# thangvubk/SoftGroup

Hardware: AMD Instinct MI355X
Metric: scans/sec ScanNet-v2-like inference (softgroup_scannet.yaml, full forward_test) (higher is better)
Workload: dtype f32

## Files before the change

### softgroup_amd/csrc/bfs.hip

```cpp
#include <stdlib.h>

#include <atomic>
#include <map>
#include <mutex>
#include <utility>

#include "common.h"
#include "scan.h"

namespace sg {

constexpr int kCap = SG_BALLQUERY_MAX_NEIGHBORS;
constexpr int kEmitThreads = 512;
constexpr int kEmitWaves = kEmitThreads / 64;

#define SG_LD(p) __hip_atomic_load((p), __ATOMIC_RELAXED, __HIP_MEMORY_SCOPE_AGENT)
#define SG_ST(p, v) __hip_atomic_store((p), (v), __ATOMIC_RELAXED, __HIP_MEMORY_SCOPE_AGENT)

struct BfsWs {
  int32_t *parent, *lab, *size, *cid, *coff, *owner, *seeds, *ebase, *wcnt, *asym_nodes;
  int4 *label;
  int2 *erec;
  int32_t *counters;
  void *scan_ws;
  size_t scan_bytes;
  int32_t *big_stage[2];
  unsigned long long *big_rec[2];
};

constexpr int kBigFastWgs = 16;
constexpr int kBigSlice = 8192;
constexpr int kBigClusterMin = 16384;
inline bool big_fast_on() {
  const char *e = getenv("SG_BFS_BIG_FAST");
  return !(e && atoi(e) == 0);
}
inline int thin_levels_on() {
  const char *e = getenv("SG_BFS_THIN");
  return e ? atoi(e) : 0;
}
inline bool big_local_on() {
  const char *e = getenv("SG_BFS_BIG_LOCAL");
  return !(e && atoi(e) == 0);
}
inline size_t big_stage_entries(int n) {
  return n > kBigClusterMin && big_fast_on() ? static_cast<size_t>(n) + static_cast<size_t>(kBigFastWgs) * kBigSlice : 0;
}

static bool bfs_carve(void *ws, size_t ws_bytes, int n, int64_t n_edges, BfsWs *w) {
  Workspace a(ws, ws_bytes);
  const size_t nn = static_cast<size_t>(n > 0 ? n : 1);
  w->parent = a.take<int32_t>(nn);
  w->lab = a.take<int32_t>(nn);
  w->label = a.take<int4>(nn);
  w->size = a.take<int32_t>(nn);
  w->cid = a.take<int32_t>(nn);
  w->coff = a.take<int32_t>(nn);
  w->owner = a.take<int32_t>(nn);
  w->seeds = a.take<int32_t>(nn);
  w->ebase = a.take<int32_t>(nn);
  w->wcnt = a.take<int32_t>(nn);
  w->asym_nodes = a.take<int32_t>(nn);
  w->counters = a.take<int32_t>(64);
  w->scan_bytes = scan_workspace_bytes(n);
  w->scan_ws = a.take<char>(w->scan_bytes);
  w->erec = a.take<int2>(static_cast<size_t>(n_edges > 0 ? n_edges : 1));
  bool ok = w->scan_ws != nullptr && w->erec != nullptr;
  const size_t be = big_stage_entries(n);
  for (int i = 0; i < 2; ++i) {
    w->big_stage[i] = be ? a.take<int32_t>(be) : nullptr;
    w->big_rec[i] = be ? a.take<unsigned long long>(be) : nullptr;
    ok = ok && (be == 0 || (w->big_stage[i] != nullptr && w->big_rec[i] != nullptr));
// ... 4 lines not shown
__device__ __forceinline__ int uf_find(int32_t *parent, int x) {
  int cur = SG_LD(&parent[x]);
  if (cur != x) {
    int prev = x, next;
    while (cur > (next = SG_LD(&parent[cur]))) {
      SG_ST(&parent[prev], next);
      prev = cur;
      cur = next;
    }
  }
  return cur;
}

__device__ __forceinline__ void uf_union(int32_t *parent, int a, int b) {
  while (a != b) {
    if (a < b) { const int t = a; a = b; b = t; }
    const int old = atomicCAS(&parent[a], a, b);
    if (old == a) return;
    a = uf_find(parent, old);
    b = uf_find(parent, b);
  }
}

__device__ __forceinline__ bool list_has_sorted(const int32_t *__restrict__ lst, int len, int key) {
  int lo = 0, hi = len;
  while (lo < hi) {
    const int mid = (lo + hi) >> 1;
    const int v = lst[mid];
    if (v < key) lo = mid + 1; else hi = mid;
  }
  return lo < len && lst[lo] == key;
}

__global__ void __launch_bounds__(256) bfs_init_kernel(int n, int32_t *parent, int32_t *size,
                                                      int32_t *owner) {
  const int i = blockIdx.x * 256 + threadIdx.x;
  if (i < n) {
    parent[i] = i;
    size[i] = 0;
    owner[i] = 0x7fffffff;
  }
}

constexpr int kSample = 2;
template <int SAMPLE, int G>
__global__ void __launch_bounds__(256) bfs_union_kernel(const int32_t *__restrict__ idx,
                                                       const int32_t *__restrict__ start_len, int n,
                                                       int lists_sorted, int radius_lists,
                                                       int32_t *parent, int32_t *asym_nodes,
                                                       int32_t *counters) {
  constexpr int kNodes = 64 / G;
  const int wave = threadIdx.x >> 6, lane = group_lane<G>(), sub = (threadIdx.x & 63) / G;
  for (int u0 = (blockIdx.x * 4 + wave) * kNodes; u0 < n; u0 += gridDim.x * 4 * kNodes) {
    const int u = u0 + sub;
    const bool live = G == 64 || u < n;
    const int st = live ? start_len[2 * u] : 0, ln_all = live ? start_len[2 * u + 1] : 0;
    const int ln = SAMPLE ? min(ln_all, kSample) : ln_all;
    const bool u_capped = ln_all >= kCap;
    bool any_asym = false;
    const int ru = SAMPLE || !live ? -1 : SG_LD(&parent[u]);
    for (int p0 = 0; p0 < ln; p0 += G) {
      const int p = p0 + lane;
      const int v = p < ln ? idx[st + p] : u;
      bool sym = true;
      if (v != u) {
        const int vst = start_len[2 * v], vln = start_len[2 * v + 1];
        if (!radius_lists || u_capped || vln >= kCap) {
          if (lists_sorted) {
            sym = list_has_sorted(idx + vst, vln, u);
          } else {
            sym = false;
            for (int j = 0; j < vln; ++j)
              if (idx[vst + j] == u) { sym = true; break; }
          }
        }
        if (sym) {
          if (v < u && (SAMPLE || SG_LD(&parent[v]) != ru)) uf_union(parent, uf_find(parent, u), uf_find(parent, v));
        }
      }
      any_asym |= !sym;
    }
    if (!SAMPLE && group_any<G>(any_asym)) {
      if (lane == 0) asym_nodes[atomicAdd(&counters[0], 1)] = u;
    }
  }
}

__global__ void __launch_bounds__(256) bfs_hook_min_kernel(const int32_t *__restrict__ idx,
                                                          const int32_t *__restrict__ start_len, int n,
                                                          int lists_sorted, int radius_lists, int32_t *parent) {
  const int u = blockIdx.x * 256 + threadIdx.x;
  if (u >= n) return;
  const int st = start_len[2 * u], ln = start_len[2 * u + 1];
  if (ln == 0 || !lists_sorted) return;
  const int v = idx[st];
  if (v >= u) return;
  if (!radius_lists || ln >= kCap || start_len[2 * v + 1] >= kCap)
    if (!list_has_sorted(idx + start_len[2 * v], start_len[2 * v + 1], u)) return;
  parent[u] = v;
}
__global__ void __launch_bounds__(256) bfs_compress_kernel(int n, int32_t *parent) {
  const int i = blockIdx.x * 256 + threadIdx.x;
  if (i < n) SG_ST(&parent[i], uf_find(parent, i));
}

__global__ void __launch_bounds__(256) bfs_flatten_kernel(int n, int32_t *parent, int32_t *lab) {
  const int i = blockIdx.x * 256 + threadIdx.x;
  if (i >= n) return;
  int r = i;
  while (true) {
    const int p = SG_LD(&parent[r]);
    if (p == r) break;
    r = p;
  }
  lab[i] = r;
}
__global__ void __launch_bounds__(256) bfs_store_root_kernel(int n, const int32_t *__restrict__ lab,
                                                            int32_t *__restrict__ parent) {
  const int i = blockIdx.x * 256 + threadIdx.x;
  if (i < n) parent[i] = lab[i];
}

template <int G>
__global__ void __launch_bounds__(256) bfs_propagate_kernel(const int32_t *__restrict__ idx,
                                                           const int32_t *__restrict__ start_len,
                                                           const int32_t *__restrict__ asym_nodes,
                                                           int n_asym,
                                                           const int32_t *__restrict__ root_of,
                                                           int32_t *lab, int32_t *counters) {
  const int lane = group_lane<G>();
  for (int a = (blockIdx.x * 256 + threadIdx.x) / G; a < n_asym; a += (gridDim.x * 256) / G) {
    const int u = asym_nodes[a];
    const int ru = root_of[u];
    const int st = start_len[2 * u], ln = start_len[2 * u + 1];
    for (int p = lane; p < ln; p += G) {
      const int rv = root_of[idx[st + p]];
      if (rv == ru) continue;
      const int lu = SG_LD(&lab[ru]);
      if (lu < SG_LD(&lab[rv])) {
        if (atomicMin(&lab[rv], lu) > lu) SG_ST(&counters[1], 1);
      }
    }
  }
}

__global__ void __launch_bounds__(256) bfs_label_kernel(int n, const int32_t *__restrict__ root_of,
                                                       const int32_t *__restrict__ lab,
                                                       const int32_t *__restrict__ start_len,
                                                       int4 *__restrict__ node_rec, int32_t *size) {
  const int i = blockIdx.x * 256 + threadIdx.x;
  const bool valid = i < n;
  const int l = valid ? lab[root_of[i]] : -1;
  int rank = 0, peers = 0, my_leader = threadIdx.x & 63;
// ... 67 lines not shown
      erec[rv.z + p] = rt.x == rv.x ? make_int2(min(rt.y, 0xfffe) | (rt.w << 16), rt.z)
                                    : make_int2(0xffff, 0);
    }
  }
}

__device__ __forceinline__ void lds_prefetch_b32(const void *gsrc, unsigned lds_dst) {
  unsigned keep;
  asm volatile("s_mov_b32 %0, m0\n\ts_mov_b32 m0, %2\n\ts_nop 0\n\tglobal_load_lds_dword %1, off\n\t"
               "s_mov_b32 m0, %0"
               : "=&s"(keep) : "v"(gsrc), "s"(lds_dst) : "memory");
}

__device__ __forceinline__ int wg_excl_scan(int v, int *lds, int *total) {
  const int w = threadIdx.x >> 6, l = threadIdx.x & 63;
  const int incl = wave_incl_scan(v);
  if (l == 63) lds[w] = incl;
  __syncthreads();
  int carry = 0, tot = 0;
#pragma unroll
  for (int i = 0; i < kEmitWaves; ++i) {
    const int x = lds[i];
    if (i < w) carry += x;
    tot += x;
  }
  __syncthreads();
  *total = tot;
  return carry + incl - v;
}

constexpr int kOwnCap = 16384;
constexpr int kFrontChunk = 1024;
constexpr int kE2 = 4096;
constexpr int kThinIter = 8;
constexpr int kThinEdges = 64 * kThinIter;
static_assert(kThinEdges <= kFrontChunk, "a thin level's winners must fit the LDS frontier");

__global__ void __launch_bounds__(kEmitThreads) bfs_emit_kernel(
    const int32_t *__restrict__ idx, const int32_t *__restrict__ start_len,
    const int4 *__restrict__ node_rec, const int2 *__restrict__ erec,
    const int32_t *__restrict__ seeds, const int32_t *__restrict__ cluster_offsets, int n_cluster,
    int32_t *owner_g, int32_t *cluster_idxs, int32_t *stats, int skip_above, int only_above,
    const int32_t *gate ,
    int thin_mode ) {
  const bool thin_on = thin_mode != 0, thin_prefetch = thin_mode == 2;
  if (gate != nullptr && SG_LD(gate) == 0) return;
  __shared__ int lds_scan[kEmitWaves];
  __shared__ int own_lds[kOwnCap];
  __shared__ int f_st[2][kFrontChunk], f_ln[2][kFrontChunk];
  __shared__ int f_eb[kFrontChunk], f_wc[kFrontChunk];
  __shared__ unsigned short ebuf[kE2];
  __shared__ int e_st[kE2], e_g[kE2];
  __shared__ unsigned short e_ln[kE2];
  __shared__ int pf_sink[kEmitThreads];
  __shared__ unsigned char thin_map[kThinEdges];
  __shared__ int thin_state[8];
  const int wave = threadIdx.x >> 6, lane = threadIdx.x & 63;
  const unsigned pf_dst = __builtin_amdgcn_readfirstlane(
      static_cast<unsigned>(reinterpret_cast<uintptr_t>(pf_sink + wave * 64)));
  static_assert(sizeof(int2) == 8, "edge records are 8 bytes: 16 per 128-byte line");
  for (int c = blockIdx.x; c < n_cluster; c += gridDim.x) {
    const int seed = seeds[c];
    const int off = cluster_offsets[c];
    const int size = cluster_offsets[c + 1] - off;
    if (size > skip_above || size <= only_above) continue;
    const bool own_in_lds = size <= kOwnCap;
    int32_t *Q = cluster_idxs + 2LL * off;
    if (own_in_lds)
      for (int i = threadIdx.x; i < size; i += kEmitThreads) own_lds[i] = 0x7fffffff;
    __syncthreads();
    if (threadIdx.x == 0) {
      const int4 rec = node_rec[seed];
      SG_ST(&Q[0], c);
      SG_ST(&Q[1], seed);
      if (own_in_lds) own_lds[rec.y] = -1; else SG_ST(&owner_g[seed], -1);
      f_st[0][0] = rec.z;
      f_ln[0][0] = rec.w;
    }
    asm volatile("s_waitcnt vmcnt(0)" ::: "memory");
    __syncthreads();
    auto rec2 = [&](int v) -> int2 { return *reinterpret_cast<const int2 *>(node_rec + v); };
    auto claim = [&](int v, int pos) {
      const int2 ll = rec2(v);
      if (ll.x != seed) return;
      if (own_in_lds) { if (own_lds[ll.y] > pos) atomicMin(&own_lds[ll.y], pos); }
      else if (SG_LD(&owner_g[v]) > pos) atomicMin(&owner_g[v], pos);
    };
    auto owner_of = [&](int v) -> int {
      const int2 ll = rec2(v);
      if (ll.x != seed) return -2;
      return own_in_lds ? own_lds[ll.y] : SG_LD(&owner_g[v]);
    };
    auto mark_done = [&](int v) {
      if (own_in_lds) own_lds[rec2(v).y] = -1; else SG_ST(&owner_g[v], -1);
    };
    int head = 0, tail = 1;
    int n_fast = 0, n_gen = 0, sum_e = 0, max_l = 0;
    int conv_lo = -1;
    auto convert_pending = [&]() {
      if (conv_lo < 0) return;
      for (int o = conv_lo + threadIdx.x; o < tail; o += kEmitThreads)
        SG_ST(&Q[2 * o + 1], idx[SG_LD(&Q[2 * o + 1])]);
      conv_lo = -1;
      asm volatile("s_waitcnt vmcnt(0)" ::: "memory");
      __syncthreads();
    };
    int cur = 0;
    bool in_lds = true;
    bool thin_ok = thin_on;
    while (head < tail) {
      const int L = tail - head;
      if (thin_ok && own_in_lds && in_lds && L <= 64) {
        if (wave == 0) {
          int h = head, t = tail, cu = cur, cl = conv_lo, levels = 0, edges = 0;
          while (true) {
            const int Lw = t - h;
            if (Lw <= 0 || Lw > 64) break;
            const int ln = lane < Lw ? f_ln[cu][lane] : 0;
            const int incl = wave_incl_scan(ln);
            const int E = __builtin_amdgcn_readlane(incl, 63);
            if (E > kThinEdges) break;
            const int eb = incl - ln;
            if (lane < Lw) f_eb[lane] = eb;
            for (int q = 0; q < Lw; ++q) {
              const int ln_q = __builtin_amdgcn_readlane(ln, q), eb_q = __builtin_amdgcn_readlane(eb, q);
              for (int p = lane; p < ln_q; p += 64) thin_map[eb_q + p] = static_cast<unsigned char>(q);
            }
            int2 r[kThinIter];
            int g[kThinIter];
#pragma unroll
            for (int j = 0; j < kThinIter; ++j) {
              const int e = j * 64 + lane;
              g[j] = 0;
              r[j] = make_int2(0xffff, 0);
              if (e < E) {
                const int q = thin_map[e];
                g[j] = f_st[cu][q] + (e - f_eb[q]);
                r[j] = erec[g[j]];
              }
            }
#pragma unroll
            for (int j = 0; j < kThinIter; ++j) {
              const int e = j * 64 + lane;
              const int slot = r[j].x & 0xffff;
              if (e < E && slot != 0xffff) {
                const int cur_owner = own_lds[slot];
                if (cur_owner > e) atomicMin(&own_lds[slot], e);
                if (thin_prefetch && cur_owner >= 0) {
                  const int tl = r[j].x >> 16;
                  const char *first = reinterpret_cast<const char *>(erec + r[j].y);
                  const char *last = reinterpret_cast<const char *>(erec + r[j].y + max(tl, 1) - 1);
                  const uintptr_t l0 = reinterpret_cast<uintptr_t>(first) & ~static_cast<uintptr_t>(127);
                  const int nlines = static_cast<int>(((reinterpret_cast<uintptr_t>(last) & ~static_cast<uintptr_t>(127)) - l0) >> 7) + 1;
                  for (int k = 0; k < 4; ++k)
                    if (k < nlines) lds_prefetch_b32(reinterpret_cast<const void *>(l0 + 128u * k), pf_dst);
                }
              }
            }
            const int nxt = cu ^ 1;
            int t_new = 0;
#pragma unroll
            for (int j = 0; j < kThinIter; ++j) {
              const int e = j * 64 + lane;
              const int slot = r[j].x & 0xffff;
              const bool win = e < E && slot != 0xffff && own_lds[slot] == e;
              const uint64_t bal = __ballot(win);
              if (win) {
                const int oo = t_new + mask_prefix(bal);
                SG_ST(&Q[2 * (t + oo)], c);
                SG_ST(&Q[2 * (t + oo) + 1], g[j]);
                f_st[nxt][oo] = r[j].y;
                f_ln[nxt][oo] = r[j].x >> 16;
                own_lds[slot] = -1;
              }
              t_new += __popcll(bal);
            }
            if (cl < 0 && t_new > 0) cl = t;
            h = t;
            t += t_new;
            cu = nxt;
            ++levels;
            edges += E;
          }
          asm volatile("s_waitcnt vmcnt(0)" ::: "memory");
          if (lane == 0) {
            thin_state[0] = h; thin_state[1] = t; thin_state[2] = cu; thin_state[3] = cl;
            thin_state[4] = levels; thin_state[5] = edges;
          }
        }
        __syncthreads();
        const int levels = thin_state[4];
        head = thin_state[0];
        tail = thin_state[1];
        cur = thin_state[2];
        conv_lo = thin_state[3];
        n_fast += levels;
        sum_e += thin_state[5];
        max_l = max(max_l, L);
        __syncthreads();
        in_lds = true;
        thin_ok = false;
        if (levels > 0) continue;
      }
      thin_ok = thin_on;
      int E = -1;
      if (in_lds && L <= kFrontChunk) {
        int carry = 0;
        for (int b0 = 0; b0 < L; b0 += kEmitThreads) {
          const int q = b0 + threadIdx.x;
          const int ln = q < L ? f_ln[cur][q] : 0;
          int tot;
          const int ex = wg_excl_scan(ln, lds_scan, &tot);
          if (q < L) f_eb[q] = carry + ex;
          carry += tot;
        }
        __syncthreads();
        E = carry;
      }
      if (E >= 0 && E <= kE2) {
        ++n_fast; sum_e += E; max_l = max(max_l, L);
        for (int e = threadIdx.x; e < E; e += kEmitThreads) {
          int lo = 0, hi = L;
          while (hi - lo > 1) {
            const int mid = (lo + hi) >> 1;
            if (f_eb[mid] <= e) lo = mid; else hi = mid;
          }
          const int g = f_st[cur][lo] + (e - f_eb[lo]);
          const int2 r = erec[g];
          const unsigned short slot = static_cast<unsigned short>(r.x & 0xffff);
          ebuf[e] = slot;
          e_g[e] = g;
          e_st[e] = r.y;
          e_ln[e] = static_cast<unsigned short>(r.x >> 16);
          if (slot != 0xffffu) {
            if (own_in_lds) {
              const int cur_owner = own_lds[slot];
              if (cur_owner > e) atomicMin(&own_lds[slot], e);
              if (cur_owner >= 0) {
                const int tl = r.x >> 16;
                const char *first = reinterpret_cast<const char *>(erec + r.y);
                const char *last = reinterpret_cast<const char *>(erec + r.y + max(tl, 1) - 1);
                const uintptr_t l0 = reinterpret_cast<uintptr_t>(first) & ~static_cast<uintptr_t>(127);
                const int nlines = static_cast<int>(((reinterpret_cast<uintptr_t>(last) & ~static_cast<uintptr_t>(127)) - l0) >> 7) + 1;
                for (int j = 0; j < 4; ++j)
                  if (j < nlines) lds_prefetch_b32(reinterpret_cast<const void *>(l0 + 128u * j), pf_dst);
              }
            } else {
              const int v = idx[g];
              if (SG_LD(&owner_g[v]) > e) atomicMin(&owner_g[v], e);
            }
          }
        }
        if (!own_in_lds) asm volatile("s_waitcnt vmcnt(0)" ::: "memory");
        __syncthreads();
        const int nxt = cur ^ 1;
        int t_new = 0;
        for (int b0 = 0; b0 < E; b0 += kEmitThreads) {
          const int e = b0 + threadIdx.x;
          unsigned short slot = 0xffffu;
          bool win = false;
          int v = 0;
          if (e < E) {
            slot = ebuf[e];
            if (slot != 0xffffu) {
              if (own_in_lds) {
                win = own_lds[slot] == e;
              } else {
                v = idx[e_g[e]];
                win = SG_LD(&owner_g[v]) == e;
              }
            }
          }
          int tot;
          const int oo = t_new + wg_excl_scan(win ? 1 : 0, lds_scan, &tot);
          if (win) {
            SG_ST(&Q[2 * (tail + oo)], c);
            SG_ST(&Q[2 * (tail + oo) + 1], e_g[e]);
            if (oo < kFrontChunk) {
              f_st[nxt][oo] = e_st[e];
              f_ln[nxt][oo] = e_ln[e];
            }
            if (own_in_lds) own_lds[slot] = -1; else SG_ST(&owner_g[v], -1);
          }
          t_new += tot;
        }
        if (conv_lo < 0 && t_new > 0) conv_lo = tail;
        if (!own_in_lds) asm volatile("s_waitcnt vmcnt(0)" ::: "memory");
        __syncthreads();
        head = tail;
        tail += t_new;
        cur = nxt;
        in_lds = t_new <= kFrontChunk;
        continue;
      }
      ++n_gen; max_l = max(max_l, L);
      convert_pending();
      auto stage = [&](int ch, int carry_in) -> int {
        const int q0 = ch * kFrontChunk, cnt = min(kFrontChunk, L - q0);
        int carry = carry_in;
        for (int b0 = 0; b0 < cnt; b0 += kEmitThreads) {
          const int q = b0 + threadIdx.x;
          int ln = 0;
          if (q < cnt) {
            const int4 rec = node_rec[SG_LD(&Q[2 * (head + q0 + q) + 1])];
            f_st[0][q] = rec.z;
            ln = rec.w;
            f_ln[0][q] = ln;
          }
          int tot;
          const int ex = wg_excl_scan(ln, lds_scan, &tot);
          if (q < cnt) f_eb[q] = carry + ex;
          carry += tot;
        }
        __syncthreads();
        return carry;
      };
      const int n_chunks = (L + kFrontChunk - 1) / kFrontChunk;
      int carry = 0;
      for (int ch = 0; ch < n_chunks; ++ch) {
        carry = stage(ch, carry);
        const int cnt = min(kFrontChunk, L - ch * kFrontChunk);
        for (int q = wave; q < cnt; q += kEmitWaves) {
          const int st = f_st[0][q], ln = f_ln[0][q], base = f_eb[q];
          for (int p = lane; p < ln; p += 64) claim(idx[st + p], base + p);
        }
        __syncthreads();
      }
      asm volatile("s_waitcnt vmcnt(0)" ::: "memory");
      __syncthreads();
      int appended = 0;
      carry = 0;
      for (int ch = 0; ch < n_chunks; ++ch) {
        carry = stage(ch, carry);
        const int cnt = min(kFrontChunk, L - ch * kFrontChunk);
        for (int q = wave; q < cnt; q += kEmitWaves) {
          const int st = f_st[0][q], ln = f_ln[0][q], base = f_eb[q];
          int wins = 0;
          for (int p0 = 0; p0 < ln; p0 += 64) {
            const int p = p0 + lane;
            wins += __popcll(__ballot(p < ln && owner_of(idx[st + p]) == base + p));
          }
          if (lane == 0) f_wc[q] = wins;
        }
        __syncthreads();
        int chunk_new = 0;
        for (int b0 = 0; b0 < cnt; b0 += kEmitThreads) {
          const int q = b0 + threadIdx.x;
          const int w_ = q < cnt ? f_wc[q] : 0;
          int tot;
          const int ex = wg_excl_scan(w_, lds_scan, &tot);
          if (q < cnt) f_wc[q] = chunk_new + ex;
          chunk_new += tot;
        }
        __syncthreads();
        for (int q = wave; q < cnt; q += kEmitWaves) {
          const int st = f_st[0][q], ln = f_ln[0][q], base = f_eb[q];
          int obase = tail + appended + f_wc[q];
          for (int p0 = 0; p0 < ln; p0 += 64) {
            const int p = p0 + lane;
            int v = 0;
            bool win = false;
            if (p < ln) {
              v = idx[st + p];
              win = owner_of(v) == base + p;
            }
            const uint64_t bal = __ballot(win);
            if (win) {
              const int o = obase + mask_prefix(bal);
              SG_ST(&Q[2 * o], c);
              SG_ST(&Q[2 * o + 1], v);
            }
            obase += __popcll(bal);
          }
        }
        appended += chunk_new;
        __syncthreads();
      }
      asm volatile("s_waitcnt vmcnt(0)" ::: "memory");
      __syncthreads();
      for (int o = tail + threadIdx.x; o < tail + appended; o += kEmitThreads)
        mark_done(SG_LD(&Q[2 * o + 1]));
      const bool keep = own_in_lds && appended <= kFrontChunk;
      if (keep)
        for (int o = threadIdx.x; o < appended; o += kEmitThreads) {
          const int4 rec = node_rec[SG_LD(&Q[2 * (tail + o) + 1])];
          f_st[0][o] = rec.z;
          f_ln[0][o] = rec.w;
        }
      asm volatile("s_waitcnt vmcnt(0)" ::: "memory");
      __syncthreads();
      head = tail;
      tail += appended;
      cur = 0;
      in_lds = keep;
    }
    convert_pending();
    if (stats && threadIdx.x == 0 && c < 256) {
      stats[c * 8 + 0] = size; stats[c * 8 + 1] = n_fast; stats[c * 8 + 2] = n_gen;
      stats[c * 8 + 3] = sum_e; stats[c * 8 + 4] = max_l;
    }
    __syncthreads();
  }
}


constexpr int kBigWgsMax = 256;
constexpr int kBigMin = kOwnCap;
constexpr int kBigNodes = 1024;
constexpr int kBigEdges = 8192;
constexpr int kBigDirectDegree = 32;
static_assert(kBigSlice == kBigEdges && kBigClusterMin == kBigMin && kBfsGiantMin == kBigMin, "staging sizes follow the kernel's constants");
static_assert(kBigNodes <= 65535, "c_j holds node indices of a range as 16-bit");

__device__ __forceinline__ bool big_barrier(int32_t *bar, int &epoch, int32_t *fail, int *lds_flag) {
  asm volatile("s_waitcnt vmcnt(0)" ::: "memory");
  __syncthreads();
  if (threadIdx.x == 0) {
    __hip_atomic_fetch_add(bar, 1, __ATOMIC_RELAXED, __HIP_MEMORY_SCOPE_AGENT);
    const int target = (epoch + 1) * static_cast<int>(gridDim.x);
    unsigned spins = 0;
    int ok = 1;
    while (__hip_atomic_load(bar, __ATOMIC_RELAXED, __HIP_MEMORY_SCOPE_AGENT) < target) {
      __builtin_amdgcn_s_sleep(1);
      if ((++spins & 1023u) == 0u) {
        if (spins > (1u << 24) || __hip_atomic_load(fail, __ATOMIC_RELAXED, __HIP_MEMORY_SCOPE_AGENT)) {
          __hip_atomic_store(fail, 1, __ATOMIC_RELAXED, __HIP_MEMORY_SCOPE_AGENT);
          ok = 0;
          break;
        }
      }
    }
    *lds_flag = ok;
// ... 967 lines not shown
extern "C" {

int sg_grouping_set_lanes(int lanes) {
  SG_REQUIRE(lanes_value_ok(lanes), "sg_grouping_set_lanes: lanes must be 0, 8, 16, 32 or 64");
  grouping_lanes_forced();
  return g_group_lanes.exchange(lanes, std::memory_order_relaxed);
}

size_t sg_bfs_workspace_bytes(int n, int64_t n_edges) {
  const size_t nn = static_cast<size_t>(n > 0 ? n : 1);
  const size_t ne = static_cast<size_t>(n_edges > 0 ? n_edges : 1);
  const size_t be = big_stage_entries(n);
  return 14 * align_up(nn * 4) + align_up(64 * 4) + align_up(scan_workspace_bytes(n)) +
         align_up(ne * sizeof(int2)) + 2 * (align_up(be * 4) + align_up(be * 8)) + 256;
}

int sg_bfs_cluster_label(const int32_t *bq_idxs, const int32_t *start_len, int n, int64_t n_edges,
                         int list_flags, const int32_t *seg_of_point, const float *seg_thr,
                         int n_seg, int32_t *n_cluster_host, int32_t *sum_npoint_host, void *ws,
                         size_t ws_bytes, sg_stream_t stream_) {
  SG_REQUIRE(n >= 0 && n_seg >= 1 && seg_thr != nullptr, "sg_bfs_cluster_label: bad arguments");
  hipStream_t stream = as_stream(stream_);
  BfsWs w;
  if (!bfs_carve(ws, ws_bytes, n, n_edges, &w)) {
    set_error("sg_bfs_cluster_label: workspace too small");
    return SG_ERR_WORKSPACE;
  }
  *n_cluster_host = 0;
  *sum_npoint_host = 0;
  if (n == 0) return SG_OK;
  const int grid = (n + 255) / 256;
  const int lanes_union = lanes_auto(n_edges, n, kNarrowMeanUnion);
  const int lanes = lanes_auto(n_edges, n, kNarrowMean);
  hipMemsetAsync(w.counters, 0, 64 * 4, stream);
  bfs_init_kernel<<<grid, 256, 0, stream>>>(n, w.parent, w.size, w.owner);
  static const bool one_pass = getenv("SG_BFS_ONE_PASS") != nullptr;
  if (!one_pass) {
    static const bool sample_env = getenv("SG_BFS_SAMPLE") != nullptr;
    if (sample_env || !(list_flags & SG_LISTS_SORTED))
      launch_union<1>(lanes_union, stream, bq_idxs, start_len, n, list_flags & SG_LISTS_SORTED,
                      list_flags & SG_LISTS_RADIUS, w.parent, w.asym_nodes, w.counters);
    else
      bfs_hook_min_kernel<<<grid, 256, 0, stream>>>(bq_idxs, start_len, n, list_flags & SG_LISTS_SORTED,
                                                   list_flags & SG_LISTS_RADIUS, w.parent);
    bfs_compress_kernel<<<grid, 256, 0, stream>>>(n, w.parent);
  }
  launch_union<0>(lanes_union, stream, bq_idxs, start_len, n, list_flags & SG_LISTS_SORTED,
                  list_flags & SG_LISTS_RADIUS, w.parent, w.asym_nodes, w.counters);
  bfs_flatten_kernel<<<grid, 256, 0, stream>>>(n, w.parent, w.lab);
  bfs_store_root_kernel<<<grid, 256, 0, stream>>>(n, w.lab, w.parent);

  int32_t *host_counters = pinned_words();
  SG_REQUIRE(host_counters != nullptr, "sg_bfs_cluster_label: pinned allocation failed");
  for (int i = 0; i < 5; ++i) host_counters[i] = 0;
  for (int pass = 0; pass < 2; ++pass) {
    if (pass == 1) {
      const int n_asym = host_counters[0];
      while (true) {
        hipMemsetAsync(w.counters + 1, 0, 4, stream);
        launch_propagate(lanes, stream, bq_idxs, start_len, w.asym_nodes, n_asym, w.parent, w.lab, w.counters);
        host_counters[8] = 0;
        hipMemcpyAsync(host_counters + 8, w.counters + 1, 4, hipMemcpyDeviceToHost, stream);
        if (hipStreamSynchronize(stream) != hipSuccess) return check_launch("bfs propagate");
        if (!host_counters[8]) break;
      }
      bfs_zero_size_kernel<<<grid, 256, 0, stream>>>(n, w.size);
    }
    bfs_label_kernel<<<grid, 256, 0, stream>>>(n, w.parent, w.lab, start_len, w.label, w.size);
    const int4 *label = w.label;
    const int32_t *size = w.size;
    int32_t *cid = w.cid, *coff = w.coff;
    auto keep = [label, size, seg_of_point, seg_thr] __device__(int64_t i) -> int {
      if (label[i].x != static_cast<int32_t>(i)) return 0;
      const float thr = seg_thr[seg_of_point ? seg_of_point[i] : 0];
      return static_cast<float>(size[i]) >= thr ? 1 : 0;
    };
    int32_t *max_kept = w.counters + 4;
    auto keep_size = [keep, size, max_kept] __device__(int64_t i) -> int {
      const int s = keep(i) ? size[i] : 0;
      if (s > kBigMin) atomicMax(max_kept, s);
      return s;
    };
    int rc = exclusive_scan(keep, [cid] __device__(int64_t i, int v) { cid[i] = v; }, n,
// ... 6 lines not shown
    if (hipStreamSynchronize(stream) != hipSuccess) return check_launch("sg_bfs_cluster_label");
    if (host_counters[0] == 0) break;
    if (pass == 0) hipMemsetAsync(w.counters + 4, 0, 4, stream);
  }
  *n_cluster_host = host_counters[2];
  *sum_npoint_host = host_counters[3];
  t_bfs_note.ws = ws;
  t_bfs_note.max_kept = host_counters[4];
  return check_launch("sg_bfs_cluster_label");
}

int sg_bfs_cluster_emit(const int32_t *bq_idxs, const int32_t *start_len, int n, int64_t n_edges,
                        const int32_t *seg_of_point, const float *seg_thr, int n_cluster,
                        int sum_npoint, int32_t *cluster_idxs, int32_t *cluster_offsets, void *ws,
                        size_t ws_bytes, sg_stream_t stream_) {
  SG_REQUIRE(n >= 0 && n_cluster >= 0 && sum_npoint >= 0, "sg_bfs_cluster_emit: bad arguments");
  hipStream_t stream = as_stream(stream_);
  BfsWs w;
  if (!bfs_carve(ws, ws_bytes, n, n_edges, &w)) {
    set_error("sg_bfs_cluster_emit: workspace too small");
    return SG_ERR_WORKSPACE;
  }
  if (n_cluster == 0 || n == 0) {
    hipMemsetAsync(cluster_offsets, 0, 4, stream);
    return SG_OK;
  }
  bfs_seed_kernel<<<(n + 255) / 256, 256, 0, stream>>>(n, w.label, w.size, w.cid, w.coff,
                                                       seg_of_point, seg_thr, w.seeds,
                                                       cluster_offsets);
  launch_edge_rec(grouping_lanes_for(n_edges, n), stream, bq_idxs, w.label, w.cid, w.seeds, n, n_cluster, w.erec);
  static const bool want_stats = getenv("SG_BFS_STATS") != nullptr;
  int32_t *stats = nullptr;
  if (want_stats) {
    hipMalloc(&stats, 256 * 8 * 4);
    hipMemsetAsync(stats, 0, 256 * 8 * 4, stream);
  }
  static const bool big_on = !(getenv("SG_BFS_BIG") && atoi(getenv("SG_BFS_BIG")) == 0);
  const bool noted = t_bfs_note.ws == ws && t_bfs_note.max_kept >= 0;
  const bool has_big = big_on && n < (1 << 21) && sum_npoint > kBigMin && (!noted || t_bfs_note.max_kept > kBigMin);
  t_bfs_note.ws = nullptr;
  static const bool side_env = !(getenv("SG_BFS_BIG_SIDE") && atoi(getenv("SG_BFS_BIG_SIDE")) == 0);
  BfsSide *side = has_big && side_env && !want_stats ? bfs_side(stream) : nullptr;
  hipStream_t main_stream = stream;
  BfsDefer *defer = t_bfs_defer;
  t_bfs_defer = nullptr;
  if (defer != nullptr) defer->deferred = false;
  if (side != nullptr) {
    if (hipEventRecord(side->fork, stream) != hipSuccess || hipStreamWaitEvent(side->side, side->fork, 0) != hipSuccess) {
      set_error("sg_bfs_cluster_emit: forking the side stream failed");
      return SG_ERR_LAUNCH;
    }
  }
  bfs_emit_kernel<<<min(n_cluster, 4096), kEmitThreads, 0, stream>>>(
      bq_idxs, start_len, w.label, w.erec, w.seeds, cluster_offsets, n_cluster, w.owner, cluster_idxs,
      stats, big_on && n < (1 << 21) ? kBigMin : 0x7fffffff, -1, nullptr, thin_levels_on());
  if (side != nullptr) stream = side->side;
  if (has_big) {
    static const int big_wgs_env = getenv("SG_BFS_BIG_WGS") ? atoi(getenv("SG_BFS_BIG_WGS")) : 16;
    const int big_wgs = big_wgs_env < 8 ? 8 : big_wgs_env > kBigWgsMax ? kBigWgsMax : big_wgs_env;
    int32_t *sync = w.asym_nodes;
    static const bool flags_on = getenv("SG_BFS_BIG_FLAGS") && atoi(getenv("SG_BFS_BIG_FLAGS")) != 0;
    if (static_cast<size_t>(n) >= static_cast<size_t>(kBigSyncWords)) {
      hipMemsetAsync(sync, 0, kBigSyncWords * 4, stream);
      if (const char *e = getenv("SG_BFS_FORCE_FALLBACK"))
        if (atoi(e) & 1) hipMemsetAsync(sync + 1, 1, 1, stream);
      const int32_t *gate = nullptr;
      if (big_local_on() && big_fast_on() && w.big_stage[0] != nullptr &&
          static_cast<size_t>(n) >= static_cast<size_t>(kBigSyncWords) + 96) {
        const int lw_env = getenv("SG_BFS_BIG_LOCAL_WGS") ? atoi(getenv("SG_BFS_BIG_LOCAL_WGS")) : 16;
        const int lw = lw_env < 8 ? 8 : lw_env > kBigWgsMax ? kBigWgsMax : lw_env;
        const int every_env = getenv("SG_BFS_BIG_LOCAL_EVERY") ? atoi(getenv("SG_BFS_BIG_LOCAL_EVERY")) : 4;
        const int warm_env = getenv("SG_BFS_BIG_LOCAL_WARM") ? atoi(getenv("SG_BFS_BIG_LOCAL_WARM")) : 8;
        const int every = every_env < 1 ? 1 : every_env, warm = warm_env < 1 ? 1 : warm_env;
        const bool novis = getenv("SG_BFS_BIG_LOCAL_NOVIS") && atoi(getenv("SG_BFS_BIG_LOCAL_NOVIS")) != 0;
        int32_t *sync3 = sync + kBigSyncWords;
        const size_t rows = big_stage_entries(n) / (2 * static_cast<size_t>(lw));
        hipMemsetAsync(sync3, 0, 96 * 4, stream);
        hipMemsetAsync(w.big_rec[1], 0, rows * 2 * lw * 8, stream);
        hipMemsetD32Async(reinterpret_cast<hipDeviceptr_t>(w.parent), 0x7fffffff, n, stream);
        if (const char *e = getenv("SG_BFS_FORCE_FALLBACK"))
          if (atoi(e) & 2) hipMemsetAsync(sync3 + 1, 1, 1, stream);
        const size_t vis_bytes = (!novis && n <= kVisWords * 32) ? static_cast<size_t>((n + 31) >> 5) * 4 : 0;
        {
          static std::mutex mu;
          static uint64_t done_mask = 0;
          int dev = 0;
          hipGetDevice(&dev);
          std::lock_guard<std::mutex> g(mu);
          if (dev < 0 || dev >= 64 || !((done_mask >> dev) & 1)) {
            if (hipFuncSetAttribute(reinterpret_cast<const void *>(bfs_emit_big_local_kernel),
                                    hipFuncAttributeMaxDynamicSharedMemorySize, kVisWords * 4) != hipSuccess) {
              (void)hipGetLastError();
              set_error("sg_bfs_cluster_emit: %d bytes of dynamic LDS are not available on this device", kVisWords * 4);
              return SG_ERR_LAUNCH;
            }
            if (dev >= 0 && dev < 64) done_mask |= 1ull << dev;
          }
        }
        bfs_emit_big_local_kernel<<<lw, kEmitThreads, vis_bytes, stream>>>(
            bq_idxs, w.label, w.erec, w.seeds, cluster_offsets, n_cluster, w.owner, w.parent, w.big_stage[0],
            w.big_rec[0], w.big_rec[1], static_cast<int>(rows) - 1, cluster_idxs, sync3, novis ? 0x7fffffff : n, every, warm,
            want_stats);
        gate = sync3 + 1;
        bfs_owner_reset_kernel<<<grid_for(n, 256, 1024), 256, 0, stream>>>(n, w.label, w.size, kBigMin, gate, w.owner);
      }
      if (big_fast_on() && big_wgs <= kBigFastWgs && w.big_stage[0] != nullptr)
        bfs_emit_big_kernel<true><<<big_wgs, kEmitThreads, 0, stream>>>(
            bq_idxs, w.label, w.erec, w.seeds, cluster_offsets, n_cluster, w.owner, w.wcnt, w.big_stage[0],
            w.big_stage[1], w.big_rec[0], w.big_rec[1], n, cluster_idxs, sync, flags_on, want_stats, gate);
      else
        bfs_emit_big_kernel<false><<<big_wgs, kEmitThreads, 0, stream>>>(
            bq_idxs, w.label, w.erec, w.seeds, cluster_offsets, n_cluster, w.owner, w.wcnt, w.parent, w.lab,
            nullptr, nullptr, 0, cluster_idxs, sync, false, false, gate);
      bfs_owner_reset_kernel<<<grid_for(n, 256, 1024), 256, 0, stream>>>(n, w.label, w.size, kBigMin,
                                                                        sync + 1, w.owner);
      bfs_emit_kernel<<<min(n_cluster, 256), kEmitThreads, 0, stream>>>(
          bq_idxs, start_len, w.label, w.erec, w.seeds, cluster_offsets, n_cluster, w.owner,
          cluster_idxs, nullptr, 0x7fffffff, kBigMin, sync + 1, thin_levels_on());
    }
  }
  if (side != nullptr && defer != nullptr) {
    stream = main_stream;
    if (hipEventRecord(side->back, stream) != hipSuccess || hipStreamWaitEvent(side->side, side->back, 0) != hipSuccess) {
      set_error("sg_bfs_cluster_emit: handing the side stream over failed");
      return SG_ERR_LAUNCH;
    }
    defer->deferred = true;
    defer->side = side->side;
  } else if (side != nullptr) {
    stream = main_stream;
    if (hipEventRecord(side->join, side->side) != hipSuccess || hipStreamWaitEvent(stream, side->join, 0) != hipSuccess) {
      set_error("sg_bfs_cluster_emit: joining the side stream failed");
      return SG_ERR_LAUNCH;
    }
  }
  if (want_stats && has_big && big_local_on()) {
    hipStreamSynchronize(stream);
    int32_t h[32];
    hipMemcpy(h, w.asym_nodes + kBigSyncWords, sizeof(h), hipMemcpyDeviceToHost);
    unsigned long long lp[8];
    hipMemcpy(lp, w.asym_nodes + kBigSyncWords + 16, sizeof(lp), hipMemcpyDeviceToHost);
    const double lv = lp[5] ? static_cast<double>(lp[5]) : 1.0;
    fprintf(stderr, "bfs giant clusters, local form: %s (%d); %d clusters, %d levels (%llu re-partition levels); us per level: "
            "re-partition %.2f, edge bases+claim sweep %.2f, pool+drain %.2f, rendezvous %.2f, emit sweep %.2f, totals+publication %.2f\n",
            h[1] ? "gave up" : "completed", h[1], h[9], h[8], lp[6], lp[0] / lv / 100.0, lp[1] / lv / 100.0, lp[7] / lv / 100.0,
            lp[2] / lv / 100.0, lp[3] / lv / 100.0, lp[4] / lv / 100.0);
  }
  if (want_stats && has_big) {
    unsigned long long ph[6];
    hipStreamSynchronize(stream);
    hipMemcpy(ph, w.asym_nodes + 16, sizeof(ph), hipMemcpyDeviceToHost);
    const double lv = ph[5] ? static_cast<double>(ph[5]) : 1.0;
    fprintf(stderr, "bfs giant clusters: %llu cached levels; us per level: wait records %.2f, ranks+queue+staged records %.2f, "
            "claim sweep %.2f, claim rendezvous %.2f, emit sweep+drain %.2f\n", ph[5], ph[0] / lv / 100.0, ph[1] / lv / 100.0,
            ph[2] / lv / 100.0, ph[3] / lv / 100.0, ph[4] / lv / 100.0);
  }
  if (want_stats) {
    int32_t h[256 * 8];
    hipMemcpy(h, stats, sizeof(h), hipMemcpyDeviceToHost);
    hipFree(stats);
    for (int c = 0; c < n_cluster && c < 256; ++c)
      fprintf(stderr, "bfs cluster %d: size %d fast levels %d generic levels %d edges %d max frontier %d\n", c,
              h[c * 8], h[c * 8 + 1], h[c * 8 + 2], h[c * 8 + 3], h[c * 8 + 4]);
  }
  return check_launch("sg_bfs_cluster_emit");
}

}
```

Baseline: 429.6.

## Restructure BFS emit fast levels with register-held edges and fused init/hook kernels

Rewrites the per-cluster emit kernel's fast level path: each thread holds a contiguous run of edge records in registers, winners are compacted with one wave-scan plus cross-wave partial sums instead of per-chunk workgroup scans, and next-level edge bases are written during compaction so the frontier scan is skipped. It also removes the experimental thin-level path and its LDS buffers, and drops the global-owner branch from the fast path, so clusters whose owners do not fit in LDS now go to the generic path. On the label side, the counter memset and the min-neighbour hook are folded into the init kernel, and the store-root kernel is merged into flatten, cutting several launches. Optional per-phase timing counters are added behind the stats flag.

```diff
diff --git a/softgroup_amd/csrc/bfs.hip b/softgroup_amd/csrc/bfs.hip
--- a/softgroup_amd/csrc/bfs.hip
+++ b/softgroup_amd/csrc/bfs.hip
@@ -3,6 +3,7 @@
 #include <atomic>
 #include <map>
 #include <mutex>
+#include <type_traits>
 #include <utility>
 
 #include "common.h"
@@ -34,10 +35,6 @@
 inline bool big_fast_on() {
   const char *e = getenv("SG_BFS_BIG_FAST");
   return !(e && atoi(e) == 0);
-}
-inline int thin_levels_on() {
-  const char *e = getenv("SG_BFS_THIN");
-  return e ? atoi(e) : 0;
 }
 inline bool big_local_on() {
   const char *e = getenv("SG_BFS_BIG_LOCAL");
@@ -108,14 +105,28 @@
   return lo < len && lst[lo] == key;
 }
 
-__global__ void __launch_bounds__(256) bfs_init_kernel(int n, int32_t *parent, int32_t *size,
-                                                      int32_t *owner) {
-  const int i = blockIdx.x * 256 + threadIdx.x;
-  if (i < n) {
-    parent[i] = i;
-    size[i] = 0;
-    owner[i] = 0x7fffffff;
-  }
+template <bool HOOK>
+__global__ void __launch_bounds__(256) bfs_init_kernel(const int32_t *__restrict__ idx,
+                                                      const int32_t *__restrict__ start_len, int n, int radius_lists,
+                                                      int32_t *parent, int32_t *size, int32_t *owner,
+                                                      int32_t *counters) {
+  const int u = blockIdx.x * 256 + threadIdx.x;
+  if (u < 64) counters[u] = 0;
+  if (u >= n) return;
+  size[u] = 0;
+  owner[u] = 0x7fffffff;
+  int p = u;
+  if (HOOK) {
+    const int st = start_len[2 * u], ln = start_len[2 * u + 1];
+    const int v = ln > 0 ? idx[st] : u;
+    if (v < u) {
+      bool sym = true;
+      if (!radius_lists || ln >= kCap || start_len[2 * v + 1] >= kCap)
+        sym = list_has_sorted(idx + start_len[2 * v], start_len[2 * v + 1], u);
+      if (sym) p = v;
+    }
+  }
+  parent[u] = p;
 }
 
 constexpr int kSample = 2;
@@ -162,19 +173,6 @@
   }
 }
 
-__global__ void __launch_bounds__(256) bfs_hook_min_kernel(const int32_t *__restrict__ idx,
-                                                          const int32_t *__restrict__ start_len, int n,
-                                                          int lists_sorted, int radius_lists, int32_t *parent) {
-  const int u = blockIdx.x * 256 + threadIdx.x;
-  if (u >= n) return;
-  const int st = start_len[2 * u], ln = start_len[2 * u + 1];
-  if (ln == 0 || !lists_sorted) return;
-  const int v = idx[st];
-  if (v >= u) return;
-  if (!radius_lists || ln >= kCap || start_len[2 * v + 1] >= kCap)
-    if (!list_has_sorted(idx + start_len[2 * v], start_len[2 * v + 1], u)) return;
-  parent[u] = v;
-}
 __global__ void __launch_bounds__(256) bfs_compress_kernel(int n, int32_t *parent) {
   const int i = blockIdx.x * 256 + threadIdx.x;
   if (i < n) SG_ST(&parent[i], uf_find(parent, i));
@@ -190,11 +188,7 @@
     r = p;
   }
   lab[i] = r;
-}
-__global__ void __launch_bounds__(256) bfs_store_root_kernel(int n, const int32_t *__restrict__ lab,
-                                                            int32_t *__restrict__ parent) {
-  const int i = blockIdx.x * 256 + threadIdx.x;
-  if (i < n) parent[i] = lab[i];
+  SG_ST(&parent[i], r);
 }
 
 template <int G>
@@ -328,29 +322,22 @@
 constexpr int kOwnCap = 16384;
 constexpr int kFrontChunk = 1024;
 constexpr int kE2 = 4096;
-constexpr int kThinIter = 8;
-constexpr int kThinEdges = 64 * kThinIter;
-static_assert(kThinEdges <= kFrontChunk, "a thin level's winners must fit the LDS frontier");
+constexpr int kFastRun = kE2 / kEmitThreads;
+constexpr int kEmitStatWords = 16;
 
 __global__ void __launch_bounds__(kEmitThreads) bfs_emit_kernel(
     const int32_t *__restrict__ idx, const int32_t *__restrict__ start_len,
     const int4 *__restrict__ node_rec, const int2 *__restrict__ erec,
     const int32_t *__restrict__ seeds, const int32_t *__restrict__ cluster_offsets, int n_cluster,
     int32_t *owner_g, int32_t *cluster_idxs, int32_t *stats, int skip_above, int only_above,
-    const int32_t *gate ,
-    int thin_mode ) {
-  const bool thin_on = thin_mode != 0, thin_prefetch = thin_mode == 2;
+    const int32_t *gate ) {
   if (gate != nullptr && SG_LD(gate) == 0) return;
   __shared__ int lds_scan[kEmitWaves];
+  __shared__ int2 lds_part[2][kEmitWaves];
   __shared__ int own_lds[kOwnCap];
-  __shared__ int f_st[2][kFrontChunk], f_ln[2][kFrontChunk];
-  __shared__ int f_eb[kFrontChunk], f_wc[kFrontChunk];
-  __shared__ unsigned short ebuf[kE2];
-  __shared__ int e_st[kE2], e_g[kE2];
-  __shared__ unsigned short e_ln[kE2];
+  __shared__ int f_st[2][kFrontChunk], f_ln[2][kFrontChunk], f_eb[2][kFrontChunk];
+  __shared__ int f_wc[kFrontChunk];
   __shared__ int pf_sink[kEmitThreads];
-  __shared__ unsigned char thin_map[kThinEdges];
-  __shared__ int thin_state[8];
   const int wave = threadIdx.x >> 6, lane = threadIdx.x & 63;
   const unsigned pf_dst = __builtin_amdgcn_readfirstlane(
       static_cast<unsigned>(reinterpret_cast<uintptr_t>(pf_sink + wave * 64)));
@@ -372,6 +359,7 @@
       if (own_in_lds) own_lds[rec.y] = -1; else SG_ST(&owner_g[seed], -1);
       f_st[0][0] = rec.z;
       f_ln[0][0] = rec.w;
+      f_eb[0][0] = 0;
     }
     asm volatile("s_waitcnt vmcnt(0)" ::: "memory");
     __syncthreads();
@@ -392,6 +380,15 @@
     };
     int head = 0, tail = 1;
     int n_fast = 0, n_gen = 0, sum_e = 0, max_l = 0;
+    unsigned ph0 = 0, ph1 = 0, ph2 = 0, ph3 = 0;
+    unsigned long long t_prev = 0;
+    auto tick = [&](unsigned &acc) {
+      if (stats != nullptr) {
+        const unsigned long long now = __builtin_amdgcn_s_memrealtime();
+        acc += static_cast<unsigned>(now - t_prev);
+        t_prev = now;
+      }
+    };
     int conv_lo = -1;
     auto convert_pending = [&]() {
       if (conv_lo < 0) return;
@@ -403,191 +400,131 @@
     };
     int cur = 0;
     bool in_lds = true;
-    bool thin_ok = thin_on;
+    bool have_eb = true;
+    int E = f_ln[0][0];
+    auto scan_frontier = [&](int L) -> int {
+      int carry = 0;
+      for (int b0 = 0; b0 < L; b0 += kEmitThreads) {
+        const int q = b0 + threadIdx.x;
+        const int ln = q < L ? f_ln[cur][q] : 0;
+        int tot;
+        const int ex = wg_excl_scan(ln, lds_scan, &tot);
+        if (q < L) f_eb[cur][q] = carry + ex;
+        carry += tot;
+      }
+      __syncthreads();
+      return carry;
+    };
+    auto fast_level = [&](auto kmax, const int K) {
+      constexpr int KM = decltype(kmax)::value;
+      const int L = tail - head;
+      if (stats != nullptr) t_prev = __builtin_amdgcn_s_memrealtime();
+      const int e0 = threadIdx.x * K;
+      int2 r[KM];
+      int g[KM];
+      int lo = 0;
+      if (e0 < E) {
+        int hi = L;
+        while (hi - lo > 1) {
+          const int mid = (lo + hi) >> 1;
+          if (f_eb[cur][mid] <= e0) lo = mid; else hi = mid;
+        }
+      }
+#pragma unroll
+      for (int j = 0; j < KM; ++j) {
+        const int e = e0 + j;
+        g[j] = 0;
+        r[j] = make_int2(0xffff, 0);
+        if (j < K && e < E) {
+          if (KM > 1)
+            while (lo + 1 < L && f_eb[cur][lo + 1] <= e) ++lo;
+          g[j] = f_st[cur][lo] + (e - f_eb[cur][lo]);
+          r[j] = erec[g[j]];
+        }
+      }
+#pragma unroll
+      for (int j = 0; j < KM; ++j) {
+        const int e = e0 + j;
+        const int slot = r[j].x & 0xffff;
+        if (slot != 0xffff) {
+          const int cur_owner = own_lds[slot];
+          if (cur_owner > e) atomicMin(&own_lds[slot], e);
+          if (cur_owner >= 0) {
+            const int tl = r[j].x >> 16;
+            const char *first = reinterpret_cast<const char *>(erec + r[j].y);
+            const char *last = reinterpret_cast<const char *>(erec + r[j].y + max(tl, 1) - 1);
+            const uintptr_t l0 = reinterpret_cast<uintptr_t>(first) & ~static_cast<uintptr_t>(127);
+            const int nlines = static_cast<int>(((reinterpret_cast<uintptr_t>(last) & ~static_cast<uintptr_t>(127)) - l0) >> 7) + 1;
+            for (int k = 0; k < 4; ++k)
+              if (k < nlines) lds_prefetch_b32(reinterpret_cast<const void *>(l0 + 128u * k), pf_dst);
+          }
+        }
+      }
+      tick(ph0);
+      __syncthreads();
+      tick(ph1);
+      unsigned wmask = 0;
+      int wins = 0, lens = 0;
+#pragma unroll
+      for (int j = 0; j < KM; ++j) {
+        const int slot = r[j].x & 0xffff;
+        if (slot != 0xffff && own_lds[slot] == e0 + j) {
+          wmask |= 1u << j;
+          ++wins;
+          lens += r[j].x >> 16;
+        }
+      }
+      const int incl_w = wave_incl_scan(wins), incl_l = wave_incl_scan(lens);
+      if (lane == 63) lds_part[cur][wave] = make_int2(incl_w, incl_l);
+      __syncthreads();
+      int oo = incl_w - wins, eb = incl_l - lens, t_new = 0, e_new = 0;
+#pragma unroll
+      for (int i = 0; i < kEmitWaves; ++i) {
+        const int2 x = lds_part[cur][i];
+        if (i < wave) { oo += x.x; eb += x.y; }
+        t_new += x.x;
+        e_new += x.y;
+      }
+      tick(ph2);
+      const int nxt = cur ^ 1;
+#pragma unroll
+      for (int j = 0; j < KM; ++j) {
+        if ((wmask >> j) & 1u) {
+          const int tl = r[j].x >> 16;
+          SG_ST(&Q[2 * (tail + oo)], c);
+          SG_ST(&Q[2 * (tail + oo) + 1], g[j]);
+          if (oo < kFrontChunk) {
+            f_st[nxt][oo] = r[j].y;
+            f_ln[nxt][oo] = tl;
+            f_eb[nxt][oo] = eb;
+          }
+          own_lds[r[j].x & 0xffff] = -1;
+          ++oo;
+          eb += tl;
+        }
+      }
+      if (conv_lo < 0 && t_new > 0) conv_lo = tail;
+      __syncthreads();
+      tick(ph3);
+      head = tail;
+      tail += t_new;
+      cur = nxt;
+      in_lds = t_new <= kFrontChunk;
+      E = e_new;
+    };
     while (head < tail) {
       const int L = tail - head;
-      if (thin_ok && own_in_lds && in_lds && L <= 64) {
-        if (wave == 0) {
-          int h = head, t = tail, cu = cur, cl = conv_lo, levels = 0, edges = 0;
-          while (true) {
-            const int Lw = t - h;
-            if (Lw <= 0 || Lw > 64) break;
-            const int ln = lane < Lw ? f_ln[cu][lane] : 0;
-            const int incl = wave_incl_scan(ln);
-            const int E = __builtin_amdgcn_readlane(incl, 63);
-            if (E > kThinEdges) break;
-            const int eb = incl - ln;
-            if (lane < Lw) f_eb[lane] = eb;
-            for (int q = 0; q < Lw; ++q) {
-              const int ln_q = __builtin_amdgcn_readlane(ln, q), eb_q = __builtin_amdgcn_readlane(eb, q);
-              for (int p = lane; p < ln_q; p += 64) thin_map[eb_q + p] = static_cast<unsigned char>(q);
-            }
-            int2 r[kThinIter];
-            int g[kThinIter];
-#pragma unroll
-            for (int j = 0; j < kThinIter; ++j) {
-              const int e = j * 64 + lane;
-              g[j] = 0;
-              r[j] = make_int2(0xffff, 0);
-              if (e < E) {
-                const int q = thin_map[e];
-                g[j] = f_st[cu][q] + (e - f_eb[q]);
-                r[j] = erec[g[j]];
-              }
-            }
-#pragma unroll
-            for (int j = 0; j < kThinIter; ++j) {
-              const int e = j * 64 + lane;
-              const int slot = r[j].x & 0xffff;
-              if (e < E && slot != 0xffff) {
-                const int cur_owner = own_lds[slot];
-                if (cur_owner > e) atomicMin(&own_lds[slot], e);
-                if (thin_prefetch && cur_owner >= 0) {
-                  const int tl = r[j].x >> 16;
-                  const char *first = reinterpret_cast<const char *>(erec + r[j].y);
-                  const char *last = reinterpret_cast<const char *>(erec + r[j].y + max(tl, 1) - 1);
-                  const uintptr_t l0 = reinterpret_cast<uintptr_t>(first) & ~static_cast<uintptr_t>(127);
-                  const int nlines = static_cast<int>(((reinterpret_cast<uintptr_t>(last) & ~static_cast<uintptr_t>(127)) - l0) >> 7) + 1;
-                  for (int k = 0; k < 4; ++k)
-                    if (k < nlines) lds_prefetch_b32(reinterpret_cast<const void *>(l0 + 128u * k), pf_dst);
-                }
-              }
-            }
-            const int nxt = cu ^ 1;
-            int t_new = 0;
-#pragma unroll
-            for (int j = 0; j < kThinIter; ++j) {
-              const int e = j * 64 + lane;
-              const int slot = r[j].x & 0xffff;
-              const bool win = e < E && slot != 0xffff && own_lds[slot] == e;
-              const uint64_t bal = __ballot(win);
-              if (win) {
-                const int oo = t_new + mask_prefix(bal);
-                SG_ST(&Q[2 * (t + oo)], c);
-                SG_ST(&Q[2 * (t + oo) + 1], g[j]);
-                f_st[nxt][oo] = r[j].y;
-                f_ln[nxt][oo] = r[j].x >> 16;
-                own_lds[slot] = -1;
-              }
-              t_new += __popcll(bal);
-            }
-            if (cl < 0 && t_new > 0) cl = t;
-            h = t;
-            t += t_new;
-            cu = nxt;
-            ++levels;
-            edges += E;
-          }
-          asm volatile("s_waitcnt vmcnt(0)" ::: "memory");
-          if (lane == 0) {
-            thin_state[0] = h; thin_state[1] = t; thin_state[2] = cu; thin_state[3] = cl;
-            thin_state[4] = levels; thin_state[5] = edges;
-          }
-        }
-        __syncthreads();
-        const int levels = thin_state[4];
-        head = thin_state[0];
-        tail = thin_state[1];
-        cur = thin_state[2];
-        conv_lo = thin_state[3];
-        n_fast += levels;
-        sum_e += thin_state[5];
-        max_l = max(max_l, L);
-        __syncthreads();
-        in_lds = true;
-        thin_ok = false;
-        if (levels > 0) continue;
-      }
-      thin_ok = thin_on;
-      int E = -1;
-      if (in_lds && L <= kFrontChunk) {
-        int carry = 0;
-        for (int b0 = 0; b0 < L; b0 += kEmitThreads) {
-          const int q = b0 + threadIdx.x;
-          const int ln = q < L ? f_ln[cur][q] : 0;
-          int tot;
-          const int ex = wg_excl_scan(ln, lds_scan, &tot);
-          if (q < L) f_eb[q] = carry + ex;
-          carry += tot;
-        }
-        __syncthreads();
-        E = carry;
-      }
-      if (E >= 0 && E <= kE2) {
-        ++n_fast; sum_e += E; max_l = max(max_l, L);
-        for (int e = threadIdx.x; e < E; e += kEmitThreads) {
-          int lo = 0, hi = L;
-          while (hi - lo > 1) {
-            const int mid = (lo + hi) >> 1;
-            if (f_eb[mid] <= e) lo = mid; else hi = mid;
-          }
-          const int g = f_st[cur][lo] + (e - f_eb[lo]);
-          const int2 r = erec[g];
-          const unsigned short slot = static_cast<unsigned short>(r.x & 0xffff);
-          ebuf[e] = slot;
-          e_g[e] = g;
-          e_st[e] = r.y;
-          e_ln[e] = static_cast<unsigned short>(r.x >> 16);
-          if (slot != 0xffffu) {
-            if (own_in_lds) {
-              const int cur_owner = own_lds[slot];
-              if (cur_owner > e) atomicMin(&own_lds[slot], e);
-              if (cur_owner >= 0) {
-                const int tl = r.x >> 16;
-                const char *first = reinterpret_cast<const char *>(erec + r.y);
-                const char *last = reinterpret_cast<const char *>(erec + r.y + max(tl, 1) - 1);
-                const uintptr_t l0 = reinterpret_cast<uintptr_t>(first) & ~static_cast<uintptr_t>(127);
-                const int nlines = static_cast<int>(((reinterpret_cast<uintptr_t>(last) & ~static_cast<uintptr_t>(127)) - l0) >> 7) + 1;
-                for (int j = 0; j < 4; ++j)
-                  if (j < nlines) lds_prefetch_b32(reinterpret_cast<const void *>(l0 + 128u * j), pf_dst);
-              }
-            } else {
-              const int v = idx[g];
-              if (SG_LD(&owner_g[v]) > e) atomicMin(&owner_g[v], e);
-            }
-          }
-        }
-        if (!own_in_lds) asm volatile("s_waitcnt vmcnt(0)" ::: "memory");
-        __syncthreads();
-        const int nxt = cur ^ 1;
-        int t_new = 0;
-        for (int b0 = 0; b0 < E; b0 += kEmitThreads) {
-          const int e = b0 + threadIdx.x;
-          unsigned short slot = 0xffffu;
-          bool win = false;
-          int v = 0;
-          if (e < E) {
-            slot = ebuf[e];
-            if (slot != 0xffffu) {
-              if (own_in_lds) {
-                win = own_lds[slot] == e;
-              } else {
-                v = idx[e_g[e]];
-                win = SG_LD(&owner_g[v]) == e;
-              }
-            }
-          }
-          int tot;
-          const int oo = t_new + wg_excl_scan(win ? 1 : 0, lds_scan, &tot);
-          if (win) {
-            SG_ST(&Q[2 * (tail + oo)], c);
-            SG_ST(&Q[2 * (tail + oo) + 1], e_g[e]);
-            if (oo < kFrontChunk) {
-              f_st[nxt][oo] = e_st[e];
-              f_ln[nxt][oo] = e_ln[e];
-            }
-            if (own_in_lds) own_lds[slot] = -1; else SG_ST(&owner_g[v], -1);
-          }
-          t_new += tot;
-        }
-        if (conv_lo < 0 && t_new > 0) conv_lo = tail;
-        if (!own_in_lds) asm volatile("s_waitcnt vmcnt(0)" ::: "memory");
-        __syncthreads();
-        head = tail;
-        tail += t_new;
-        cur = nxt;
-        in_lds = t_new <= kFrontChunk;
-        continue;
+      if (own_in_lds && in_lds) {
+        if (!have_eb) {
+          E = scan_frontier(L);
+          have_eb = true;
+        }
+        if (E <= kE2) {
+          ++n_fast; sum_e += E; max_l = max(max_l, L);
+          if (E <= kEmitThreads) fast_level(std::integral_constant<int, 1>{}, 1);
+          else fast_level(std::integral_constant<int, kFastRun>{}, (E + kEmitThreads - 1) / kEmitThreads);
+          continue;
+        }
       }
       ++n_gen; max_l = max(max_l, L);
       convert_pending();
@@ -605,7 +542,7 @@
           }
           int tot;
           const int ex = wg_excl_scan(ln, lds_scan, &tot);
-          if (q < cnt) f_eb[q] = carry + ex;
+          if (q < cnt) f_eb[0][q] = carry + ex;
           carry += tot;
         }
         __syncthreads();
@@ -617,7 +554,7 @@
         carry = stage(ch, carry);
         const int cnt = min(kFrontChunk, L - ch * kFrontChunk);
         for (int q = wave; q < cnt; q += kEmitWaves) {
-          const int st = f_st[0][q], ln = f_ln[0][q], base = f_eb[q];
+          const int st = f_st[0][q], ln = f_ln[0][q], base = f_eb[0][q];
           for (int p = lane; p < ln; p += 64) claim(idx[st + p], base + p);
         }
         __syncthreads();
@@ -630,7 +567,7 @@
         carry = stage(ch, carry);
         const int cnt = min(kFrontChunk, L - ch * kFrontChunk);
         for (int q = wave; q < cnt; q += kEmitWaves) {
-          const int st = f_st[0][q], ln = f_ln[0][q], base = f_eb[q];
+          const int st = f_st[0][q], ln = f_ln[0][q], base = f_eb[0][q];
           int wins = 0;
           for (int p0 = 0; p0 < ln; p0 += 64) {
             const int p = p0 + lane;
@@ -650,7 +587,7 @@
         }
         __syncthreads();
         for (int q = wave; q < cnt; q += kEmitWaves) {
-          const int st = f_st[0][q], ln = f_ln[0][q], base = f_eb[q];
+          const int st = f_st[0][q], ln = f_ln[0][q], base = f_eb[0][q];
           int obase = tail + appended + f_wc[q];
           for (int p0 = 0; p0 < ln; p0 += 64) {
             const int p = p0 + lane;
@@ -689,11 +626,13 @@
       tail += appended;
       cur = 0;
       in_lds = keep;
+      have_eb = false;
     }
     convert_pending();
     if (stats && threadIdx.x == 0 && c < 256) {
-      stats[c * 8 + 0] = size; stats[c * 8 + 1] = n_fast; stats[c * 8 + 2] = n_gen;
-      stats[c * 8 + 3] = sum_e; stats[c * 8 + 4] = max_l;
+      int32_t *s = stats + c * kEmitStatWords;
+      s[0] = size; s[1] = n_fast; s[2] = n_gen; s[3] = sum_e; s[4] = max_l;
+      s[5] = static_cast<int>(ph0); s[6] = static_cast<int>(ph1); s[7] = static_cast<int>(ph2); s[8] = static_cast<int>(ph3);
     }
     __syncthreads();
   }
@@ -1727,23 +1666,21 @@
   const int grid = (n + 255) / 256;
   const int lanes_union = lanes_auto(n_edges, n, kNarrowMeanUnion);
   const int lanes = lanes_auto(n_edges, n, kNarrowMean);
-  hipMemsetAsync(w.counters, 0, 64 * 4, stream);
-  bfs_init_kernel<<<grid, 256, 0, stream>>>(n, w.parent, w.size, w.owner);
   static const bool one_pass = getenv("SG_BFS_ONE_PASS") != nullptr;
-  if (!one_pass) {
-    static const bool sample_env = getenv("SG_BFS_SAMPLE") != nullptr;
-    if (sample_env || !(list_flags & SG_LISTS_SORTED))
+  static const bool sample_env = getenv("SG_BFS_SAMPLE") != nullptr;
+  if (one_pass || sample_env || !(list_flags & SG_LISTS_SORTED)) {
+    bfs_init_kernel<false><<<grid, 256, 0, stream>>>(bq_idxs, start_len, n, 0, w.parent, w.size, w.owner, w.counters);
+    if (!one_pass)
       launch_union<1>(lanes_union, stream, bq_idxs, start_len, n, list_flags & SG_LISTS_SORTED,
                       list_flags & SG_LISTS_RADIUS, w.parent, w.asym_nodes, w.counters);
-    else
-      bfs_hook_min_kernel<<<grid, 256, 0, stream>>>(bq_idxs, start_len, n, list_flags & SG_LISTS_SORTED,
-                                                   list_flags & SG_LISTS_RADIUS, w.parent);
-    bfs_compress_kernel<<<grid, 256, 0, stream>>>(n, w.parent);
-  }
+  } else {
+    bfs_init_kernel<true><<<grid, 256, 0, stream>>>(bq_idxs, start_len, n, list_flags & SG_LISTS_RADIUS, w.parent,
+                                                   w.size, w.owner, w.counters);
+  }
+  if (!one_pass) bfs_compress_kernel<<<grid, 256, 0, stream>>>(n, w.parent);
   launch_union<0>(lanes_union, stream, bq_idxs, start_len, n, list_flags & SG_LISTS_SORTED,
                   list_flags & SG_LISTS_RADIUS, w.parent, w.asym_nodes, w.counters);
   bfs_flatten_kernel<<<grid, 256, 0, stream>>>(n, w.parent, w.lab);
-  bfs_store_root_kernel<<<grid, 256, 0, stream>>>(n, w.lab, w.parent);
 
   int32_t *host_counters = pinned_words();
   SG_REQUIRE(host_counters != nullptr, "sg_bfs_cluster_label: pinned allocation failed");
@@ -1816,8 +1753,8 @@
   static const bool want_stats = getenv("SG_BFS_STATS") != nullptr;
   int32_t *stats = nullptr;
   if (want_stats) {
-    hipMalloc(&stats, 256 * 8 * 4);
-    hipMemsetAsync(stats, 0, 256 * 8 * 4, stream);
+    hipMalloc(&stats, 256 * kEmitStatWords * 4);
+    hipMemsetAsync(stats, 0, 256 * kEmitStatWords * 4, stream);
   }
   static const bool big_on = !(getenv("SG_BFS_BIG") && atoi(getenv("SG_BFS_BIG")) == 0);
   const bool noted = t_bfs_note.ws == ws && t_bfs_note.max_kept >= 0;
@@ -1837,7 +1774,7 @@
   }
   bfs_emit_kernel<<<min(n_cluster, 4096), kEmitThreads, 0, stream>>>(
       bq_idxs, start_len, w.label, w.erec, w.seeds, cluster_offsets, n_cluster, w.owner, cluster_idxs,
-      stats, big_on && n < (1 << 21) ? kBigMin : 0x7fffffff, -1, nullptr, thin_levels_on());
+      stats, big_on && n < (1 << 21) ? kBigMin : 0x7fffffff, -1, nullptr);
   if (side != nullptr) stream = side->side;
   if (has_big) {
     static const int big_wgs_env = getenv("SG_BFS_BIG_WGS") ? atoi(getenv("SG_BFS_BIG_WGS")) : 16;
@@ -1900,7 +1837,7 @@
                                                                         sync + 1, w.owner);
       bfs_emit_kernel<<<min(n_cluster, 256), kEmitThreads, 0, stream>>>(
           bq_idxs, start_len, w.label, w.erec, w.seeds, cluster_offsets, n_cluster, w.owner,
-          cluster_idxs, nullptr, 0x7fffffff, kBigMin, sync + 1, thin_levels_on());
+          cluster_idxs, nullptr, 0x7fffffff, kBigMin, sync + 1);
     }
   }
   if (side != nullptr && defer != nullptr) {
@@ -1940,12 +1877,21 @@
             ph[2] / lv / 100.0, ph[3] / lv / 100.0, ph[4] / lv / 100.0);
   }
   if (want_stats) {
-    int32_t h[256 * 8];
+    int32_t h[256 * kEmitStatWords];
     hipMemcpy(h, stats, sizeof(h), hipMemcpyDeviceToHost);
     hipFree(stats);
-    for (int c = 0; c < n_cluster && c < 256; ++c)
+    int deepest = 0;
+    for (int c = 0; c < n_cluster && c < 256; ++c) {
+      const int32_t *s = h + c * kEmitStatWords;
       fprintf(stderr, "bfs cluster %d: size %d fast levels %d generic levels %d edges %d max frontier %d\n", c,
-              h[c * 8], h[c * 8 + 1], h[c * 8 + 2], h[c * 8 + 3], h[c * 8 + 4]);
+              s[0], s[1], s[2], s[3], s[4]);
+      if (s[1] > h[deepest * kEmitStatWords + 1]) deepest = c;
+    }
+    const int32_t *s = h + deepest * kEmitStatWords;
+    const double lv = s[1] ? static_cast<double>(s[1]) : 1.0;
+    fprintf(stderr, "bfs per-cluster kernel, cluster %d (most fast levels: %d, %.1f edges each); us per level: "
+            "search+records+claim %.2f, barrier 1 %.2f, winner test+scan %.2f, writes+barrier 3 %.2f\n", deepest, s[1],
+            s[3] / lv, s[5] / lv / 100.0, s[6] / lv / 100.0, s[7] / lv / 100.0, s[8] / lv / 100.0);
   }
   return check_launch("sg_bfs_cluster_emit");
 }
```

After: 433.9 (median of 6 runs). No clear change (+1.0%).
